# SerezD/vqvae-vqgan-pytorch-lightning

Measured on AMD Instinct MI355X. Metric: images/sec/node (256x256 bs=32/GPU) VQ-VAE train step, higher is better.
Workload: dtype bf16; 1 GPU; standard_vqvae cb=1024, 256x256 bs=32/GPU (encoder+VQ+decoder fwd/bwd + AdamW); yaml=example_confs/standard_vqvae.yaml, global_batch=32, parallelism=dp1, launch=hipGraph replay (fwd+bwd) + eager all-reduce + AdamW, deterministic=False

## Files before the change

include/vqk.h:

```cpp
#ifndef VQK_H_
#define VQK_H_

#include <stddef.h>
#include <stdint.h>

#ifdef __cplusplus
extern "C" {
#endif

#define VQK_F32 0
#define VQK_BF16 1

enum vqk_status {
    VQK_OK = 0,
    VQK_ERR_SHAPE = -1,
    VQK_ERR_DTYPE = -2,
    VQK_ERR_ALIGN = -3,
    VQK_ERR_LAUNCH = -4,
    VQK_ERR_ARG = -5,
    VQK_ERR_WORKSPACE = -6
};

const char* vqk_status_str(int status);
int vqk_version(void);
// ... 162 lines not shown
int vqk_ctx_set_tile_queue(vqk_ctx* ctx, void* ws, int64_t ws_bytes);
int vqk_ctx_set_deterministic(vqk_ctx* ctx, int on, void* ws, int64_t ws_bytes);
int vqk_set_tuning(const char* name, int value);
int vqk_reset_tuning(void);
int vqk_tuning_count(void);
const char* vqk_tuning_name(int i);
int vqk_conv_set_block_caps(int stream_blocks, int wgrad_blocks);
int vqk_probe_stream_add(const float* src, float* dst, int64_t bytes, int blocks, int passes, int sleep, void* stream);
int vqk_calib_fill(void* w, int64_t bytes, void* stream);
int vqk_calib_mfma(const void* w, int64_t w_bytes, float* sink, int iters, int blocks, void* stream);
int64_t vqk_calib_mfma_flops(int iters, int blocks);
int vqk_calib_copy(const void* src, void* dst, int64_t bytes, void* stream);
int vqk_conv_pack_dgrad(const float* w, void* wt, int dtype, int cout, int cin, int ksize, void* stream);
int vqk_conv2d_wgrad(int dtype, const void* x, const void* dy, float* dw, int n, int h_in, int w_in, int cin,
                     int cout, int ksize, int ups, const void* zeros, void* stream);
int64_t vqk_conv2d_wgrad_edge_ws_bytes(void);
int vqk_conv2d_wgrad_edge(int dtype, const void* x, const void* dy, float* dw, void* ws, int64_t ws_bytes, int n, int h,
                          int w, int cin, int cout, const void* zeros, void* stream);
int vqk_conv2d_wgrad_edge_true(int dtype, const void* x, const void* dy, float* dw, void* ws, int64_t ws_bytes, int n, int h,
                               int w, int cin, int cout, int thin_true, const void* zeros, void* stream);
int vqk_conv2d_thin_out(int dtype, const void* x, const void* w, const float* bias, void* y, int n, int h, int wd, int cin,
                        int cout, int act, const void* zeros, void* stream);
int vqk_colsum(int dtype, const void* x, int64_t rows, int c, float* out, void* stream);
int vqk_colsum_lead(int dtype, const void* x, int64_t rows, int c, int c_out, float scale, float* out, void* stream);
int vqk_cast(const float* src, void* dst, int dtype, int64_t n, void* stream);

int vqk_gn_stats(int dtype, const void* x, int n, int64_t hw, int c, int groups, float eps,
                 double* acc, float* stats, void* stream);
int vqk_gn_apply(int dtype, const void* x, const float* stats, const float* w, const float* b, void* y,
                 int n, int64_t hw, int c, int groups, int silu, void* stream);
int vqk_gn_forward(int dtype, const void* x, const float* w, const float* b, void* y, float* stats, double* ws, int n,
                   int64_t hw, int c, int groups, float eps, int silu, void* stream);
int vqk_gn_forward_presummed(int dtype, const void* x, const float* w, const float* b, void* y, float* stats, double* ws,
                             int n, int64_t hw, int c, int groups, float eps, int silu, void* stream);
int vqk_gn_forward_presummed_parts(int dtype, const void* x, const float* w, const float* b, void* y, float* stats,
// ... 130 lines not shown
```

vqvae-vqgan-pytorch-lightning_amd/_native.py:

```python
from __future__ import annotations

import ctypes
import fcntl
import os
import subprocess
from ctypes import c_char_p, c_double, c_float, c_int, c_int32, c_int64, c_void_p, POINTER

_HERE = os.path.dirname(os.path.abspath(__file__))
_CSRC = os.path.join(_HERE, 'csrc')
_SO = os.environ.get('VQK_LIB') or os.path.join(_HERE, 'libvqk.so')
_lib = None

P = c_void_p
I, L, F = c_int, c_int64, c_float

_PROTOS = {
    'vqk_row_sqnorm_f32': [P, L, I, P, P],
    'vqk_vq_assign_f32': [P, P, P, P, L, I, I, I, P, P],
    'vqk_vq_assign_filtered_f32': [P, P, P, P, L, I, I, I, P, P, L, P],
    'vqk_probe_stream_add': [P, P, L, I, I, I, P],
    'vqk_calib_fill': [P, L, P],
    'vqk_calib_mfma': [P, L, P, I, I, P],
    'vqk_calib_copy': [P, P, L, P],
    'vqk_vq_prepare_f32': [P, I, I, P, L, P],
# ... 51 lines not shown
    'vqk_conv_pack_weights': [P, P, I, I, I, I, I, I, P],
    'vqk_conv_pack_multi': [P, I, I, P],
    'vqk_conv_set_variant': [I],
    'vqk_conv_set_block_caps': [I, I],
    'vqk_set_deterministic': [I, P, L],
    'vqk_set_scratch': [P, L],
    'vqk_set_tile_queue': [P, L],
    'vqk_ctx_create': [P],
    'vqk_ctx_destroy': [P],
    'vqk_ctx_make_current': [P],
    'vqk_ctx_set_scratch': [P, P, L],
    'vqk_ctx_set_tile_queue': [P, P, L],
    'vqk_ctx_set_deterministic': [P, I, P, L],
    'vqk_conv_pack_dgrad': [P, P, I, I, I, I, P],
    'vqk_conv2d_wgrad': [I, P, P, P, I, I, I, I, I, I, I, P, P],
    'vqk_conv2d_wgrad_pooled_dy': [I, P, P, P, I, I, I, I, I, F, P, P],
    'vqk_conv2d_wgrad_ups_phase': [I, P, P, P, I, I, I, I, I, F, P, P],
    'vqk_split_pair_f32': [P, P, L, I, P],
    'vqk_conv2d_fprop_x3_gnstats': [P, P, P, P, P, I, I, I, I, I, I, P, I, P, P],
    'vqk_conv2d_wgrad_x3': [P, P, P, I, I, I, I, I, I, F, P, P],
    'vqk_conv2d_wgrad_x3_f32': [P, P, P, I, I, I, I, I, I, F, P],
    'vqk_conv2d_wgrad_pooled_dy_phase': [I, P, P, P, I, I, I, I, I, F, P, P],
    'vqk_conv2d_wgrad_edge': [I, P, P, P, P, L, I, I, I, I, I, P, P],
    'vqk_conv2d_wgrad_edge_true': [I, P, P, P, P, L, I, I, I, I, I, I, P, P],
    'vqk_conv2d_thin_out': [I, P, P, P, P, I, I, I, I, I, I, P, P],
    'vqk_colsum': [I, P, L, I, P, P],
    'vqk_colsum_lead': [I, P, L, I, I, F, P, P],
    'vqk_cast': [P, P, I, L, P],
    'vqk_gn_stats': [I, P, I, L, I, I, F, P, P, P],
    'vqk_gn_apply': [I, P, P, P, P, P, I, L, I, I, I, P],
    'vqk_gn_forward': [I, P, P, P, P, P, P, I, L, I, I, F, I, P],
    'vqk_gn_forward_presummed': [I, P, P, P, P, P, P, I, L, I, I, F, I, P],
    'vqk_gn_forward_presummed_parts': [I, P, P, P, P, P, P, I, P, I, L, I, I, F, I, P],
    'vqk_gn_backward': [I, P, P, P, P, P, P, P, P, P, I, L, I, I, I, I, P, P],
    'vqk_gn_backward_pooled_add': [I, P, P, P, P, P, P, P, P, P, I, I, I, I, I, I, P, F, P],
    'vqk_gn_backward_ws': [I, P, P, P, P, P, P, P, P, P, L, I, I, I, I, I, I, I, P, P, F, P],
    'vqk_gn_cluster_timeouts': [P],
    'vqk_gn_backward_colsum': [I, P, P, P, P, P, P, P, P, P, L, I, I, I, I, I, I, I, P, P, P],
    'vqk_pool2x2': [I, P, P, I, I, I, I, F, P],
# ... 124 lines not shown
```

vqvae-vqgan-pytorch-lightning_amd/csrc/api.cpp:

```cpp
#include <stdint.h>
#include <new>
#include "common.h"

extern "C" {

const char* vqk_status_str(int status) {
    switch (status) {
        case VQK_OK: return "ok";
        case VQK_ERR_SHAPE: return "unsupported or inconsistent shape";
        case VQK_ERR_DTYPE: return "unsupported dtype";
        case VQK_ERR_ALIGN: return "pointer is not 16-byte aligned";
        case VQK_ERR_LAUNCH: return "kernel launch failed";
        case VQK_ERR_ARG: return "bad argument";
        case VQK_ERR_WORKSPACE: return "workspace too small";
        default: return "unknown status";
    }
}

int vqk_version(void) { return 1; }
const char* vqk_arch(void) { return "gfx950"; }

}

struct vqk_ctx {
// ... 96 lines not shown
    {"GN_NO_SMALL", 0, 0},
    {"WGMX_COEF_E4", 0, 0},
    {"GN_CLUSTER_MAX_HW", 0, 0},
    {"COMM_CUS", 0, 0},
    {"MX_QUARTER", 0, 0},
    {"MX_S2", 0, 0},
    {"MX_S2_DGRAD_MIN", 0, 0},
    {"VQ_LDS", 0, 0},
    {"UPS_MERGE", 0, 0},
    {"TILE_QUEUE", 0, 0},
    {"X3_WL", 0, 0},
    {"X3_WGRAD_COEF_E4", 0, 0},
    {"X3_WGRAD_FOLD", 0, 0},
    {"X3_WGRAD_PHASE", 0, 0},
    {"X3_WGRAD_PHASE_CAP_PCT", 0, 0},
    {"X3_WGRAD_PHASE_COEF_E4", 0, 0}
};
static constexpr int kTune = (int)(sizeof(g_tune) / sizeof(g_tune[0]));
TuneSlot* tune_slot(const char* name) {
    for (int i = 0; i < kTune; ++i)
        if (strcmp(g_tune[i].name, name) == 0) return &g_tune[i];
    abort();
}
}

extern "C" int vqk_set_tuning(const char* name, int value) {
    if (!name) return VQK_ERR_ARG;
    for (int i = 0; i < vqkd::kTune; ++i)
        if (strcmp(vqkd::g_tune[i].name, name) == 0) {
            __atomic_store_n(&vqkd::g_tune[i].value, value, __ATOMIC_RELAXED);
            __atomic_store_n(&vqkd::g_tune[i].is_set, 1, __ATOMIC_RELEASE);
// ... 14 lines not shown
```

vqvae-vqgan-pytorch-lightning_amd/csrc/conv_edge.hip:

```cpp
#include "conv_geom.h"

namespace {

__device__ __forceinline__ void glds16(const void* src, char* lds_wave_base) {
    __builtin_amdgcn_global_load_lds((const VQK_GLB void*)src, (VQK_LDS void*)lds_wave_base, 16, 0, 0);
}

typedef __attribute__((ext_vector_type(8))) short s16x8;

template <int PITCH, bool SWZ>
__device__ __forceinline__ bf16x8_t tr_frag(const char* tile, int k0, int cbase, int lane) {
    const int i = lane & 15, grp = (lane >> 4) & 1, kgrp = lane >> 5;
    const int col = cbase + 16 * grp + 4 * (i & 3);
    const int row = k0 + 8 * kgrp + (i >> 2);
    const char* p0;
    if (SWZ) p0 = tile + row * PITCH + (((col >> 3) ^ ((row & 3) << 2)) << 4) + ((col & 7) << 1);
    else p0 = tile + row * PITCH + col * 2;
    const char* p1 = p0 + 4 * PITCH;
    const s16x4 lo = __builtin_amdgcn_ds_read_tr16_b64_v4i16((VQK_LDS s16x4*)p0);
    const s16x4 hi = __builtin_amdgcn_ds_read_tr16_b64_v4i16((VQK_LDS s16x4*)p1);
    const s16x8 v = {lo[0], lo[1], lo[2], lo[3], hi[0], hi[1], hi[2], hi[3]};
    return __builtin_bit_cast(bf16x8_t, v);
}

constexpr int EDGE_CW = 128;
constexpr int EDGE_PIX = 128;
constexpr int EDGE_WIDE_B = EDGE_PIX * EDGE_CW * 2;
constexpr int EDGE_IM_PITCH = 144;
constexpr int EDGE_IM_B = EDGE_PIX * EDGE_IM_PITCH;
constexpr int EDGE_STAGE = EDGE_WIDE_B + EDGE_IM_B;
constexpr int EDGE_LDS = 3 * EDGE_STAGE + 4096;
constexpr int EDGE_OUT = EDGE_CW * 72;

template <int MODE>
__global__ __launch_bounds__(256, 1) void conv3x3_wgrad_thin_kernel(const bf16_raw* __restrict__ wide,
                                                                    const bf16_raw* __restrict__ thin,
                                                                    float* __restrict__ ws, const char* __restrict__ zeros,
                                                                    int n, int h, int w) {
    extern __shared__ __attribute__((aligned(16))) char smem[];
    const int tid = threadIdx.x, lane = tid & 63;
    const int wave = __builtin_amdgcn_readfirstlane(tid >> 6);
    const int total = (int)(((int64_t)n * h * w) / EDGE_PIX);
    const int G = (int)gridDim.x, b = (int)blockIdx.x;
    const int cnt = (total - b + G - 1) / G;
    const int hw = h * w;
    constexpr int SGN = MODE == 0 ? 1 : -1;

    int s_ry[5], s_rx[5], s_ty[5], s_tx[5];
#pragma unroll
// ... 22 lines not shown
#pragma unroll
        for (int t = 0; t < 5; ++t) {
            const int q = wave + 4 * t;
            if (q < 18) {
                const int yy = y0 + s_ry[t] + s_ty[t], xx = x0 + s_rx[t] + s_tx[t];
                const void* src = zeros;
                if ((unsigned)yy < (unsigned)h && (unsigned)xx < (unsigned)w)
                    src = timg + ((int64_t)yy * w + xx) * 8;
                glds16(src, st + EDGE_WIDE_B + q * 1024);
            } else {
                glds16(zeros, smem + 3 * EDGE_STAGE + wave * 1024);
            }
        }
    };

    f32x16 acc[3];
#pragma unroll
    for (int j = 0; j < 3; ++j)
#pragma unroll
        for (int r = 0; r < 16; ++r) acc[j][r] = 0.0f;

    if (cnt > 0) issue(b, 0);
    if (cnt > 1) issue(b + G, 1);
    for (int i = 0; i < cnt; ++i) {
        if (i + 1 < cnt) asm volatile("s_waitcnt vmcnt(13)" ::: "memory");
        else asm volatile("s_waitcnt vmcnt(0)" ::: "memory");
        __syncthreads();
        if (i + 2 < cnt) issue(b + (i + 2) * G, (i + 2) % 3);
        const char* st = smem + (i % 3) * EDGE_STAGE;
#pragma unroll
        for (int k0 = 0; k0 < EDGE_PIX; k0 += 16) {
            const bf16x8_t a = tr_frag<EDGE_CW * 2, true>(st, k0, 32 * wave, lane);
#pragma unroll
            for (int j = 0; j < 3; ++j) {
                const bf16x8_t bj = tr_frag<EDGE_IM_PITCH, false>(st + EDGE_WIDE_B, k0, 32 * j, lane);
                acc[j] = __builtin_amdgcn_mfma_f32_32x32x16_bf16(a, bj, acc[j], 0, 0, 0);
            }
        }
    }
    float* part = ws + (int64_t)b * EDGE_OUT;
#pragma unroll
    for (int j = 0; j < 3; ++j) {
        const int col = 32 * j + (lane & 31);
        if (col >= 72) continue;
        const int tap = col >> 3, t = col & 7;
#pragma unroll
        for (int r = 0; r < 16; ++r) {
            const int wc = 32 * wave + (r & 3) + 8 * (r >> 2) + 4 * (lane >> 5);
            const int idx = MODE == 0 ? (wc * 9 + tap) * 8 + t : (t * 9 + tap) * EDGE_CW + wc;
            part[idx] = acc[j][r];
        }
    }
}

__global__ __launch_bounds__(256) void wgrad_thin_reduce_kernel(const float* __restrict__ ws, float* __restrict__ dw, int blocks,
                                                                int thin_true, int thin_in) {
    __shared__ float part[16][17];
    const int o = threadIdx.x & 15, kg = threadIdx.x >> 4;
    const int i = (int)blockIdx.x * 16 + o;
    float v[16];
#pragma unroll
    for (int j = 0; j < 16; ++j) {
        const int k = kg * 16 + j;
        v[j] = k < blocks ? ws[(int64_t)k * EDGE_OUT + i] : 0.0f;
    }
    float s = 0.0f;
#pragma unroll
    for (int j = 0; j < 16; ++j) s += v[j];
    part[kg][o] = s;
    __syncthreads();
    if (threadIdx.x < 16) {
        float t = 0.0f;
#pragma unroll
        for (int g2 = 0; g2 < 16; ++g2) t += part[g2][threadIdx.x];
        const int i2 = (int)blockIdx.x * 16 + (int)threadIdx.x;
        if (thin_true >= 8) dw[i2] += t;
        else if (thin_in) { const int ci = i2 & 7; if (ci < thin_true) dw[(i2 >> 3) * thin_true + ci] += t; }
        else if (i2 < thin_true * 9 * EDGE_CW) dw[i2] += t;
    }
}


constexpr int TO_TH = 8, TO_TW = 32, TO_HW2 = TO_TW + 2, TO_HPIX = (TO_TH + 2) * TO_HW2;
constexpr int TO_PITCH = 144, TO_PIECES = 48, TO_STAGE = TO_PIECES * 1024, TO_LDS = 2 * TO_STAGE;
typedef __attribute__((ext_vector_type(4))) unsigned int eu32x4;
typedef __attribute__((ext_vector_type(2))) unsigned int eu32x2;

__global__ __launch_bounds__(256, 1) void conv3x3_thin_out_kernel(const bf16_raw* __restrict__ x, const bf16_raw* __restrict__ wgt,
                                                                  const float* __restrict__ bias, bf16_raw* __restrict__ y,
                                                                  const char* __restrict__ zeros, int n, int h, int w, int act) {
    extern __shared__ __attribute__((aligned(16))) char smem[];
// ... 94 lines not shown
                    if (act == 1) v[e] = tanhf(v[e]);
                }
                const int yy = cur.y0 + 2 * wave + (gq >> 1), xx = cur.x0 + 16 * (gq & 1) + px;
                const eu32x2 o = {vqkd::pack_bf16x2(v[0], v[1]), vqkd::pack_bf16x2(v[2], v[3])};
                *reinterpret_cast<eu32x2*>(y + (((int64_t)cur.img * h + yy) * w + xx) * 8 + 4 * kq) = o;
            }
        }
        cur = nxt;
    }
}

}

extern "C" {

int64_t vqk_conv2d_wgrad_edge_ws_bytes(void) { return (int64_t)256 * EDGE_OUT * 4; }

int vqk_conv2d_wgrad_edge(int dtype, const void* x, const void* dy, float* dw, void* ws, int64_t ws_bytes, int n, int h,
                          int w, int cin, int cout, const void* zeros, void* stream) {
    return vqk_conv2d_wgrad_edge_true(dtype, x, dy, dw, ws, ws_bytes, n, h, w, cin, cout, 8, zeros, stream);
}

int vqk_conv2d_wgrad_edge_true(int dtype, const void* x, const void* dy, float* dw, void* ws, int64_t ws_bytes, int n, int h,
                               int w, int cin, int cout, int thin_true, const void* zeros, void* stream) {
    VQK_REQUIRE(x && dy && dw && ws && zeros, VQK_ERR_ARG);
    VQK_REQUIRE(thin_true >= 1 && thin_true <= 8, VQK_ERR_ARG);
    VQK_REQUIRE(vqk_aligned16(x) && vqk_aligned16(dy) && vqk_aligned16(ws) && vqk_aligned16(zeros), VQK_ERR_ALIGN);
    VQK_REQUIRE(dtype == VQK_BF16, VQK_ERR_DTYPE);
    VQK_REQUIRE(n > 0 && h > 0 && w > 0, VQK_ERR_SHAPE);
    const bool first = cin == 8 && cout == EDGE_CW, last = cout == 8 && cin == EDGE_CW;
    const int64_t m = (int64_t)n * h * w;
    VQK_REQUIRE((first || last) && ((int64_t)h * w) % EDGE_PIX == 0 && (w % EDGE_PIX == 0 || EDGE_PIX % w == 0) && m < 0x7fffffffLL,
                VQK_ERR_SHAPE);
    const int total = (int)(m / EDGE_PIX);
    int blocks = total < 256 ? total : 256;
    VQK_REQUIRE(ws_bytes >= (int64_t)blocks * EDGE_OUT * 4, VQK_ERR_ARG);
    hipStream_t st = vqk_stream(stream);
    if (first) {
        static const hipError_t attr = hipFuncSetAttribute((const void*)conv3x3_wgrad_thin_kernel<0>,
                                                           hipFuncAttributeMaxDynamicSharedMemorySize, EDGE_LDS);
        if (attr != hipSuccess) return VQK_ERR_LAUNCH;
        hipLaunchKernelGGL(conv3x3_wgrad_thin_kernel<0>, dim3((unsigned)blocks), dim3(256), EDGE_LDS, st, (const bf16_raw*)dy,
                           (const bf16_raw*)x, (float*)ws, (const char*)zeros, n, h, w);
    } else {
        static const hipError_t attr = hipFuncSetAttribute((const void*)conv3x3_wgrad_thin_kernel<1>,
                                                           hipFuncAttributeMaxDynamicSharedMemorySize, EDGE_LDS);
        if (attr != hipSuccess) return VQK_ERR_LAUNCH;
        hipLaunchKernelGGL(conv3x3_wgrad_thin_kernel<1>, dim3((unsigned)blocks), dim3(256), EDGE_LDS, st, (const bf16_raw*)x,
                           (const bf16_raw*)dy, (float*)ws, (const char*)zeros, n, h, w);
    }
    VQK_CHECK_LAUNCH();
    static_assert(EDGE_OUT % 16 == 0, "reduce blocks own 16 outputs");
    hipLaunchKernelGGL(wgrad_thin_reduce_kernel, dim3(EDGE_OUT / 16), dim3(256), 0, st, (const float*)ws, dw, blocks, thin_true, first ? 1 : 0);
    VQK_CHECK_LAUNCH();
    return VQK_OK;
}

int vqk_conv2d_thin_out(int dtype, const void* x, const void* w, const float* bias, void* y, int n, int h, int wd, int cin,
                        int cout, int act, const void* zeros, void* stream) {
    VQK_REQUIRE(x && w && y && zeros, VQK_ERR_ARG);
    VQK_REQUIRE(vqk_aligned16(x) && vqk_aligned16(w) && vqk_aligned16(y) && vqk_aligned16(zeros), VQK_ERR_ALIGN);
    VQK_REQUIRE(dtype == VQK_BF16, VQK_ERR_DTYPE);
    VQK_REQUIRE(act == 0 || act == 1, VQK_ERR_ARG);
    VQK_REQUIRE(n > 0 && cin == 128 && cout == 8 && h > 0 && wd > 0 && (h % TO_TH) == 0 && (wd % TO_TW) == 0 &&
                (int64_t)n * h * wd * 128 * 2 < 0x7fffffff0LL, VQK_ERR_SHAPE);
    const int total = n * (h / TO_TH) * (wd / TO_TW);
    const int blocks = total < 256 ? total : 256;
    static const hipError_t attr = hipFuncSetAttribute((const void*)conv3x3_thin_out_kernel,
// ... 10 lines not shown
```

vqvae-vqgan-pytorch-lightning_amd/ops.py:

```python
from __future__ import annotations

import os
import threading
import weakref

import numpy as _np
import torch

from . import _native

F32, BF16 = 0, 1
_CL = torch.channels_last


def dcode(dtype: torch.dtype) -> int:
    if dtype == torch.float32:
        return F32
    if dtype == torch.bfloat16:
        return BF16
    raise RuntimeError(f'vqk: unsupported dtype {dtype}')


def epc(dtype: torch.dtype) -> int:
    return 4 if dtype == torch.float32 else 8
# ... 722 lines not shown
    return _tagged((tensor,), lambda: tensor.backward(*args, **kwargs))


def autograd_grad(outputs, inputs, *args, **kwargs):
    roots = outputs if isinstance(outputs, (tuple, list)) else (outputs,)
    return _tagged(roots, lambda: torch.autograd.grad(outputs, inputs, *args, **kwargs))


def direct_grad(param):
    if _grad_modes()[0] and getattr(param, '_vqk_direct_grad', False) and param.grad is not None:
        return param.grad
    return None


_EDGE_WGRAD = _native.switch('VQK_EDGE_WGRAD', '1') != '0'
_EDGE_WS: dict = {}


def _edge_ws(device) -> torch.Tensor:
    _stream()
    key = _wkey(device)
    ws = _EDGE_WS.get(key)
    if ws is None:
        ws = _EDGE_WS[key] = torch.empty(_native.lib().vqk_conv2d_wgrad_edge_ws_bytes() // 4, dtype=torch.float32, device=device)
    return ws


def edge_wgrad_served(x, dy, ksize: int, ups: bool) -> bool:
    n, cin, h, w = x.shape
    return (_EDGE_WGRAD and x.dtype == torch.bfloat16 and ksize == 3 and not ups and (cin, dy.shape[1]) in ((8, 128), (128, 8))
            and (h * w) % 128 == 0 and (w % 128 == 0 or 128 % w == 0))


def raw_split_pair(t) -> torch.Tensor:
    n, c, h, w = t.shape
    out = empty_nhwc(n, 2 * c, h, w, torch.bfloat16, t.device)
    st = _timed('split_pair_kernel (HBM)', 0.0,
                lambda: _native.lib().vqk_split_pair_f32(t.data_ptr(), out.data_ptr(), n * h * w, c, _stream()), t.numel() * 8.0)
    _native.check(st, 'split_pair')
    return out


def raw_conv_wgrad(x, dy, ksize: int, ups: bool, out=None, thin_true: int = 8, x3: bool = False) -> torch.Tensor:
    n, cin, h, w = x.shape
    cout = dy.shape[1]
    dw = out if out is not None else \
        torch.zeros((cout, ksize, ksize, cin), dtype=torch.float32, device=x.device).permute(0, 3, 1, 2)
    flops = 2.0 * n * dy.shape[2] * dy.shape[3] * cout * cin * ksize * ksize
    if edge_wgrad_served(x, dy, ksize, ups):
        ws = _edge_ws(x.device)
        nbytes = (x.numel() + dy.numel()) * 2
        st = _timed('conv3x3_wgrad_thin_kernel<bf16>' + (f' {cin}->{cout}@{h}x{w}' if _EVENT_SHAPES else ''), 0.0,
                    lambda: _native.lib().vqk_conv2d_wgrad_edge_true(dcode(x.dtype), x.data_ptr(), dy.data_ptr(), dw.data_ptr(),
                                                                     ws.data_ptr(), ws.numel() * 4, n, h, w, cin, cout, int(thin_true),
                                                                     zero_page(x.device).data_ptr(), _stream()), nbytes)
        _native.check(st, 'conv2d_wgrad_edge')
        return dw
    if thin_true != 8:
        raise RuntimeError('vqk: an unpadded weight-gradient target needs the edge-conv kernel')
    if (x3 and not X3_WGRAD_FOLD and x.dtype == torch.float32 and dy.dtype == torch.float32 and ksize == 3 and cin % 64 == 0
            and cout % 64 == 0 and dy.shape[3] % 8 == 0 and dy.shape[2] % 8 == 0 and not DETERMINISTIC):
        phase = bool(ups) and X3_WGRAD_PHASE and h % 8 == 0 and w % 8 == 0
        st = _timed('conv3x3_wgrad_x3_kernel<f32 as 3 x bf16>' + (f' {cin}->{cout}@{dy.shape[2]}x{dy.shape[3]} k3{" phase" if phase else ""}' if _EVENT_SHAPES else ''), flops,
                    lambda: _native.lib().vqk_conv2d_wgrad_x3_f32(x.data_ptr(), dy.data_ptr(), dw.data_ptr(), n, h, w, cin, cout, int(ups),
                                                                  1.0, _stream()), exec_flops=3.0 * flops * (4.0 / 9.0 if phase else 1.0))
        if st != _native.ERR_SHAPE:
            _native.check(st, 'conv2d_wgrad_x3_f32')
            return dw
    if (x3 and x.dtype == torch.float32 and dy.dtype == torch.float32 and ksize == 3 and cin % 64 == 0 and cout % 64 == 0
            and dy.shape[3] % 16 == 0 and dy.shape[2] % 8 == 0 and not DETERMINISTIC and _WGMX_ON):
        xp, dyp = raw_split_pair(x), raw_split_pair(dy)
        st = _timed('conv3x3_wgrad_mx_kernel<f32 as 3 x bf16>' + (f' {cin}->{cout}@{dy.shape[2]}x{dy.shape[3]} k3' if _EVENT_SHAPES else ''), flops,
                    lambda: _native.lib().vqk_conv2d_wgrad_x3(xp.data_ptr(), dyp.data_ptr(), dw.data_ptr(), n, h, w, cin, cout, int(ups),
                                                              1.0, zero_page(x.device).data_ptr(), _stream()), exec_flops=3.0 * flops)
# ... 648 lines not shown
            n_img, _, h_out, w_out = dyc.shape
            layout = weight_layout(dt, n_img, h_out, w_out, cout_pad, cin, k, False, x3=ctx.x3)
            if ups and ctx.phase and UPS_PHASE == 1:
                dx = raw_conv_ups_phase(dyc, packed_weight(weight, cin, cout_pad, dt, k, True, phase_layout(dt, ctx.x3)), None, cin, True)
            if dx is not None:
                pass
            elif ups and can_pool_epilogue(dt, cin, layout):
                wt = packed_weight(weight, cin, cout_pad, dt, k, True, layout)
                dx = raw_conv_fprop_pooled(dyc, wt, None, None, k, False, cin, 1.0)
            else:
                wt = packed_weight(weight, cin, cout_pad, dt, k, True, layout)
                dx = raw_conv_fprop(dyc, wt, None, None, k, False, 0, dt, cin, layout)
                if ups:
                    dx = raw_pool(dx, 1.0)
        padded = cin != i or cout_pad != o
        if ctx.needs_input_grad[1]:
            tgt = None if padded else direct_grad(ctx.weight_ref)
            thin = 8
            if padded and edge_wgrad_served(x, dyc, k, ups) and (cin == i or cout_pad == o):
                tgt = direct_grad(ctx.weight_ref)
                thin = (i if cin != i else o) if tgt is not None else 8
            dw = raw_conv_wgrad(x, dyc, k, ups, out=tgt, thin_true=thin, x3=ctx.x3)
            if tgt is not None:
                dw = None
            elif padded:
                dw = dw[:o, :i]
        if has_bias and ctx.needs_input_grad[2] and id(ctx.bias_ref) in _DB_DONE:
            _DB_DONE.discard(id(ctx.bias_ref))
        elif has_bias and ctx.needs_input_grad[2]:
            n, c, h, w = dyc.shape
            tgt = direct_grad(ctx.bias_ref) if (cout_pad == c) else None
            db = raw_colsum(n * h * w, c, dyc, out=tgt, lead=o if tgt is not None else None)
            db = None if tgt is not None else db[:o]
        return dx, dw, db, dres, None, None, None, None


def conv2d(x, weight, bias=None, residual=None, ups: bool = False, act: int = 0, out_dtype=None, next_gn: int = 0):
    return Conv2dFn.apply(x, weight, bias, residual, ups, act, out_dtype, next_gn)


class GroupNormSiLUFn(torch.autograd.Function):

# ... 353 lines not shown
```

Before: 1165 images/sec.

## Add streaming 1x1 conv wgrad kernel and fuse bias-gradient sums into wgrad

Adds a new split-K MFMA kernel for 1x1 convolution weight gradients that streams pixels through LDS. It picks the pixel split heuristically and folds the partial sums, or writes atomically. Both this kernel and the thin edge 3x3 wgrad kernel now compute the bias gradient in the same pass by multiplying against a ones vector. This removes the separate colsum launch and its second read of dy. The cost is extra MFMA work and workspace, and the edge workspace size grows.

```diff
diff --git a/include/vqk.h b/include/vqk.h
--- a/include/vqk.h
+++ b/include/vqk.h
@@ -200,11 +200,16 @@
 int vqk_conv_pack_dgrad(const float* w, void* wt, int dtype, int cout, int cin, int ksize, void* stream);
 int vqk_conv2d_wgrad(int dtype, const void* x, const void* dy, float* dw, int n, int h_in, int w_in, int cin,
                      int cout, int ksize, int ups, const void* zeros, void* stream);
+int vqk_conv2d_wgrad_1x1_served(int cin, int cout);
+int vqk_conv2d_wgrad_1x1(const void* x, const void* dy, float* dw, float* db, int64_t pixels, int cin, int cout, int splits,
+                         const void* zeros, void* stream);
 int64_t vqk_conv2d_wgrad_edge_ws_bytes(void);
 int vqk_conv2d_wgrad_edge(int dtype, const void* x, const void* dy, float* dw, void* ws, int64_t ws_bytes, int n, int h,
                           int w, int cin, int cout, const void* zeros, void* stream);
 int vqk_conv2d_wgrad_edge_true(int dtype, const void* x, const void* dy, float* dw, void* ws, int64_t ws_bytes, int n, int h,
                                int w, int cin, int cout, int thin_true, const void* zeros, void* stream);
+int vqk_conv2d_wgrad_edge_db(int dtype, const void* x, const void* dy, float* dw, float* db, void* ws, int64_t ws_bytes, int n, int h,
+                             int w, int cin, int cout, int thin_true, const void* zeros, void* stream);
 int vqk_conv2d_thin_out(int dtype, const void* x, const void* w, const float* bias, void* y, int n, int h, int wd, int cin,
                         int cout, int act, const void* zeros, void* stream);
 int vqk_colsum(int dtype, const void* x, int64_t rows, int c, float* out, void* stream);
diff --git a/vqvae-vqgan-pytorch-lightning_amd/_native.py b/vqvae-vqgan-pytorch-lightning_amd/_native.py
--- a/vqvae-vqgan-pytorch-lightning_amd/_native.py
+++ b/vqvae-vqgan-pytorch-lightning_amd/_native.py
@@ -89,6 +89,8 @@
     'vqk_ctx_set_deterministic': [P, I, P, L],
     'vqk_conv_pack_dgrad': [P, P, I, I, I, I, P],
     'vqk_conv2d_wgrad': [I, P, P, P, I, I, I, I, I, I, I, P, P],
+    'vqk_conv2d_wgrad_1x1': [P, P, P, P, L, I, I, I, P, P],
+    'vqk_conv2d_wgrad_1x1_served': [I, I],
     'vqk_conv2d_wgrad_pooled_dy': [I, P, P, P, I, I, I, I, I, F, P, P],
     'vqk_conv2d_wgrad_ups_phase': [I, P, P, P, I, I, I, I, I, F, P, P],
     'vqk_split_pair_f32': [P, P, L, I, P],
@@ -98,6 +100,7 @@
     'vqk_conv2d_wgrad_pooled_dy_phase': [I, P, P, P, I, I, I, I, I, F, P, P],
     'vqk_conv2d_wgrad_edge': [I, P, P, P, P, L, I, I, I, I, I, P, P],
     'vqk_conv2d_wgrad_edge_true': [I, P, P, P, P, L, I, I, I, I, I, I, P, P],
+    'vqk_conv2d_wgrad_edge_db': [I, P, P, P, P, P, L, I, I, I, I, I, I, P, P],
     'vqk_conv2d_thin_out': [I, P, P, P, P, I, I, I, I, I, I, P, P],
     'vqk_colsum': [I, P, L, I, P, P],
     'vqk_colsum_lead': [I, P, L, I, I, F, P, P],
diff --git a/vqvae-vqgan-pytorch-lightning_amd/csrc/api.cpp b/vqvae-vqgan-pytorch-lightning_amd/csrc/api.cpp
--- a/vqvae-vqgan-pytorch-lightning_amd/csrc/api.cpp
+++ b/vqvae-vqgan-pytorch-lightning_amd/csrc/api.cpp
@@ -134,7 +134,10 @@
     {"X3_WGRAD_FOLD", 0, 0},
     {"X3_WGRAD_PHASE", 0, 0},
     {"X3_WGRAD_PHASE_CAP_PCT", 0, 0},
-    {"X3_WGRAD_PHASE_COEF_E4", 0, 0}
+    {"X3_WGRAD_PHASE_COEF_E4", 0, 0},
+    {"PIXRED_BLOCKS", 0, 0},
+    {"PIXRED_COEF", 0, 0},
+    {"PIXRED_ATOMIC", 0, 0}
 };
 static constexpr int kTune = (int)(sizeof(g_tune) / sizeof(g_tune[0]));
 TuneSlot* tune_slot(const char* name) {
diff --git a/vqvae-vqgan-pytorch-lightning_amd/csrc/conv_edge.hip b/vqvae-vqgan-pytorch-lightning_amd/csrc/conv_edge.hip
--- a/vqvae-vqgan-pytorch-lightning_amd/csrc/conv_edge.hip
+++ b/vqvae-vqgan-pytorch-lightning_amd/csrc/conv_edge.hip
@@ -31,8 +31,10 @@
 constexpr int EDGE_STAGE = EDGE_WIDE_B + EDGE_IM_B;
 constexpr int EDGE_LDS = 3 * EDGE_STAGE + 4096;
 constexpr int EDGE_OUT = EDGE_CW * 72;
-
-template <int MODE>
+constexpr int EDGE_MAXB = 256;
+constexpr int EDGE_DBW = 128;
+
+template <int MODE, bool DB>
 __global__ __launch_bounds__(256, 1) void conv3x3_wgrad_thin_kernel(const bf16_raw* __restrict__ wide,
                                                                     const bf16_raw* __restrict__ thin,
                                                                     float* __restrict__ ws, const char* __restrict__ zeros,
@@ -85,11 +87,16 @@
         }
     };
 
-    f32x16 acc[3];
+    f32x16 acc[3], accb;
 #pragma unroll
     for (int j = 0; j < 3; ++j)
 #pragma unroll
         for (int r = 0; r < 16; ++r) acc[j][r] = 0.0f;
+#pragma unroll
+    for (int r = 0; r < 16; ++r) accb[r] = 0.0f;
+    bf16x8_t ones;
+#pragma unroll
+    for (int e = 0; e < 8; ++e) ones[e] = (__bf16)1.0f;
 
     if (cnt > 0) issue(b, 0);
     if (cnt > 1) issue(b + G, 1);
@@ -106,7 +113,9 @@
             for (int j = 0; j < 3; ++j) {
                 const bf16x8_t bj = tr_frag<EDGE_IM_PITCH, false>(st + EDGE_WIDE_B, k0, 32 * j, lane);
                 acc[j] = __builtin_amdgcn_mfma_f32_32x32x16_bf16(a, bj, acc[j], 0, 0, 0);
-            }
+                if (DB && MODE == 1 && j == 1 && wave == 0) accb = __builtin_amdgcn_mfma_f32_32x32x16_bf16(ones, bj, accb, 0, 0, 0);
+            }
+            if (DB && MODE == 0) accb = __builtin_amdgcn_mfma_f32_32x32x16_bf16(a, ones, accb, 0, 0, 0);
         }
     }
     float* part = ws + (int64_t)b * EDGE_OUT;
@@ -122,18 +131,32 @@
             part[idx] = acc[j][r];
         }
     }
+    if (DB) {
+        float* pdb = ws + (int64_t)EDGE_MAXB * EDGE_OUT + (int64_t)b * EDGE_DBW;
+        if (MODE == 0) {
+            if ((lane & 31) == 0) {
+#pragma unroll
+                for (int r = 0; r < 16; ++r) pdb[32 * wave + (r & 3) + 8 * (r >> 2) + 4 * (lane >> 5)] = accb[r];
+            }
+        } else if (wave == 0 && lane < 8) {
+            pdb[lane] = accb[0];
+        }
+    }
 }
 
 __global__ __launch_bounds__(256) void wgrad_thin_reduce_kernel(const float* __restrict__ ws, float* __restrict__ dw, int blocks,
-                                                                int thin_true, int thin_in) {
+                                                                int thin_true, int thin_in, float* __restrict__ db, int db_count) {
     __shared__ float part[16][17];
     const int o = threadIdx.x & 15, kg = threadIdx.x >> 4;
-    const int i = (int)blockIdx.x * 16 + o;
+    const bool isdb = (int)blockIdx.x >= EDGE_OUT / 16;
+    const int i = (isdb ? (int)blockIdx.x - EDGE_OUT / 16 : (int)blockIdx.x) * 16 + o;
+    const float* src = isdb ? ws + (int64_t)EDGE_MAXB * EDGE_OUT : ws;
+    const int pitch = isdb ? EDGE_DBW : EDGE_OUT;
     float v[16];
 #pragma unroll
     for (int j = 0; j < 16; ++j) {
         const int k = kg * 16 + j;
-        v[j] = k < blocks ? ws[(int64_t)k * EDGE_OUT + i] : 0.0f;
+        v[j] = k < blocks ? src[(int64_t)k * pitch + i] : 0.0f;
     }
     float s = 0.0f;
 #pragma unroll
@@ -144,8 +167,9 @@
         float t = 0.0f;
 #pragma unroll
         for (int g2 = 0; g2 < 16; ++g2) t += part[g2][threadIdx.x];
-        const int i2 = (int)blockIdx.x * 16 + (int)threadIdx.x;
-        if (thin_true >= 8) dw[i2] += t;
+        const int i2 = (isdb ? (int)blockIdx.x - EDGE_OUT / 16 : (int)blockIdx.x) * 16 + (int)threadIdx.x;
+        if (isdb) { if (i2 < db_count) db[i2] += t; }
+        else if (thin_true >= 8) dw[i2] += t;
         else if (thin_in) { const int ci = i2 & 7; if (ci < thin_true) dw[(i2 >> 3) * thin_true + ci] += t; }
         else if (i2 < thin_true * 9 * EDGE_CW) dw[i2] += t;
     }
@@ -270,7 +294,7 @@
 
 extern "C" {
 
-int64_t vqk_conv2d_wgrad_edge_ws_bytes(void) { return (int64_t)256 * EDGE_OUT * 4; }
+int64_t vqk_conv2d_wgrad_edge_ws_bytes(void) { return (int64_t)EDGE_MAXB * (EDGE_OUT + EDGE_DBW) * 4; }
 
 int vqk_conv2d_wgrad_edge(int dtype, const void* x, const void* dy, float* dw, void* ws, int64_t ws_bytes, int n, int h,
                           int w, int cin, int cout, const void* zeros, void* stream) {
@@ -279,6 +303,11 @@
 
 int vqk_conv2d_wgrad_edge_true(int dtype, const void* x, const void* dy, float* dw, void* ws, int64_t ws_bytes, int n, int h,
                                int w, int cin, int cout, int thin_true, const void* zeros, void* stream) {
+    return vqk_conv2d_wgrad_edge_db(dtype, x, dy, dw, nullptr, ws, ws_bytes, n, h, w, cin, cout, thin_true, zeros, stream);
+}
+
+int vqk_conv2d_wgrad_edge_db(int dtype, const void* x, const void* dy, float* dw, float* db, void* ws, int64_t ws_bytes, int n, int h,
+                             int w, int cin, int cout, int thin_true, const void* zeros, void* stream) {
     VQK_REQUIRE(x && dy && dw && ws && zeros, VQK_ERR_ARG);
     VQK_REQUIRE(thin_true >= 1 && thin_true <= 8, VQK_ERR_ARG);
     VQK_REQUIRE(vqk_aligned16(x) && vqk_aligned16(dy) && vqk_aligned16(ws) && vqk_aligned16(zeros), VQK_ERR_ALIGN);
@@ -289,25 +318,27 @@
     VQK_REQUIRE((first || last) && ((int64_t)h * w) % EDGE_PIX == 0 && (w % EDGE_PIX == 0 || EDGE_PIX % w == 0) && m < 0x7fffffffLL,
                 VQK_ERR_SHAPE);
     const int total = (int)(m / EDGE_PIX);
-    int blocks = total < 256 ? total : 256;
-    VQK_REQUIRE(ws_bytes >= (int64_t)blocks * EDGE_OUT * 4, VQK_ERR_ARG);
+    int blocks = total < EDGE_MAXB ? total : EDGE_MAXB;
+    VQK_REQUIRE(ws_bytes >= (db ? vqk_conv2d_wgrad_edge_ws_bytes() : (int64_t)blocks * EDGE_OUT * 4), VQK_ERR_ARG);
     hipStream_t st = vqk_stream(stream);
+#define VQK_EDGE_LAUNCH(MODE, DB, WIDE, THIN)                                                                                      \
+    do {                                                                                                                          \
+        static const hipError_t attr = hipFuncSetAttribute((const void*)conv3x3_wgrad_thin_kernel<MODE, DB>,                      \
+                                                           hipFuncAttributeMaxDynamicSharedMemorySize, EDGE_LDS);                 \
+        if (attr != hipSuccess) return VQK_ERR_LAUNCH;                                                                            \
+        hipLaunchKernelGGL((conv3x3_wgrad_thin_kernel<MODE, DB>), dim3((unsigned)blocks), dim3(256), EDGE_LDS, st,                \
+                           (const bf16_raw*)(WIDE), (const bf16_raw*)(THIN), (float*)ws, (const char*)zeros, n, h, w);            \
+    } while (0)
     if (first) {
-        static const hipError_t attr = hipFuncSetAttribute((const void*)conv3x3_wgrad_thin_kernel<0>,
-                                                           hipFuncAttributeMaxDynamicSharedMemorySize, EDGE_LDS);
-        if (attr != hipSuccess) return VQK_ERR_LAUNCH;
-        hipLaunchKernelGGL(conv3x3_wgrad_thin_kernel<0>, dim3((unsigned)blocks), dim3(256), EDGE_LDS, st, (const bf16_raw*)dy,
-                           (const bf16_raw*)x, (float*)ws, (const char*)zeros, n, h, w);
+        if (db) VQK_EDGE_LAUNCH(0, true, dy, x); else VQK_EDGE_LAUNCH(0, false, dy, x);
     } else {
-        static const hipError_t attr = hipFuncSetAttribute((const void*)conv3x3_wgrad_thin_kernel<1>,
-                                                           hipFuncAttributeMaxDynamicSharedMemorySize, EDGE_LDS);
-        if (attr != hipSuccess) return VQK_ERR_LAUNCH;
-        hipLaunchKernelGGL(conv3x3_wgrad_thin_kernel<1>, dim3((unsigned)blocks), dim3(256), EDGE_LDS, st, (const bf16_raw*)x,
-                           (const bf16_raw*)dy, (float*)ws, (const char*)zeros, n, h, w);
-    }
+        if (db) VQK_EDGE_LAUNCH(1, true, x, dy); else VQK_EDGE_LAUNCH(1, false, x, dy);
+    }
+#undef VQK_EDGE_LAUNCH
     VQK_CHECK_LAUNCH();
-    static_assert(EDGE_OUT % 16 == 0, "reduce blocks own 16 outputs");
-    hipLaunchKernelGGL(wgrad_thin_reduce_kernel, dim3(EDGE_OUT / 16), dim3(256), 0, st, (const float*)ws, dw, blocks, thin_true, first ? 1 : 0);
+    static_assert(EDGE_OUT % 16 == 0 && EDGE_DBW % 16 == 0, "reduce blocks own 16 outputs");
+    hipLaunchKernelGGL(wgrad_thin_reduce_kernel, dim3(EDGE_OUT / 16 + (db ? EDGE_DBW / 16 : 0)), dim3(256), 0, st, (const float*)ws, dw,
+                       blocks, thin_true, first ? 1 : 0, db, first ? EDGE_CW : thin_true);
     VQK_CHECK_LAUNCH();
     return VQK_OK;
 }
diff --git a/vqvae-vqgan-pytorch-lightning_amd/csrc/conv_wgrad_1x1.hip b/vqvae-vqgan-pytorch-lightning_amd/csrc/conv_wgrad_1x1.hip
--- /dev/null
+++ b/vqvae-vqgan-pytorch-lightning_amd/csrc/conv_wgrad_1x1.hip
@@ -0,0 +1,265 @@
+#include "common.h"
+#include <math.h>
+
+namespace {
+
+__device__ __forceinline__ void glds16(const void* src, char* lds_wave_base) {
+    __builtin_amdgcn_global_load_lds((const VQK_GLB void*)src, (VQK_LDS void*)lds_wave_base, 16, 0, 0);
+}
+
+template <int ROWB>
+__device__ __forceinline__ bf16x8_t tr_frag(const char* tile, int k0, int cbase, int lane) {
+    constexpr int SH = ROWB == 256 ? 2 : 1;
+    const int i = lane & 15, grp = (lane >> 4) & 1, kgrp = lane >> 5;
+    const int col = cbase + 16 * grp + 4 * (i & 3);
+    const int row = k0 + 8 * kgrp + (i >> 2);
+    const int lc = col >> 3;
+    const char* p0 = tile + row * ROWB + ((lc ^ ((row & 3) << SH)) << 4) + ((col & 7) << 1);
+    const char* p1 = p0 + 4 * ROWB;
+    const s16x4 lo = __builtin_amdgcn_ds_read_tr16_b64_v4i16((VQK_LDS s16x4*)p0);
+    const s16x4 hi = __builtin_amdgcn_ds_read_tr16_b64_v4i16((VQK_LDS s16x4*)p1);
+    typedef __attribute__((ext_vector_type(8))) short s16x8;
+    const s16x8 v = {lo[0], lo[1], lo[2], lo[3], hi[0], hi[1], hi[2], hi[3]};
+    return __builtin_bit_cast(bf16x8_t, v);
+}
+
+template <int TCO, int TCI, int WM, int WN, bool DB>
+__global__ __launch_bounds__(512) void conv1x1_wgrad_stream_kernel(const bf16_raw* __restrict__ x, const bf16_raw* __restrict__ dy,
+                                                                   float* __restrict__ dw, float* __restrict__ db,
+                                                                   float* __restrict__ part, const char* __restrict__ zeros, int m,
+                                                                   int cin, int cout, int pix_per_split, int64_t slice_stride) {
+    constexpr int KP = (TCO + TCI) > 384 ? 32 : 64;
+    constexpr int KW = 8 / (WM * WN), MI = TCO / WM / 32, NJ = TCI / WN / 32;
+    constexpr int SWA = TCO < 128 ? 64 : 128, SWB = TCI < 128 ? 64 : 128;
+    constexpr int ROWBA = SWA * 2, ROWBB = SWB * 2;
+    constexpr int A_BYTES = KP * TCO * 2, B_BYTES = KP * TCI * 2, STAGE = A_BYTES + B_BYTES;
+    constexpr int PA = A_BYTES / 1024, PB = B_BYTES / 1024, NL = (PA + PB) / 8;
+    static_assert((PA + PB) % 8 == 0 && KP / 16 >= KW && MI >= 1 && NJ >= 1, "tile shape");
+    extern __shared__ __attribute__((aligned(16))) char smem[];
+    const int tid = threadIdx.x, lane = tid & 63;
+    const int wave = __builtin_amdgcn_readfirstlane(tid >> 6);
+    const int kq = wave / (WM * WN), wm = (wave % (WM * WN)) / WN, wn = wave % WN;
+    const int co0 = cout > TCO ? (int)blockIdx.x * TCO : 0;
+    const int ci0 = cin > TCI ? (int)blockIdx.x * TCI : 0;
+    const int p_begin = (int)blockIdx.y * pix_per_split;
+    const int p_end = min(m, p_begin + pix_per_split);
+    const int nsteps = (p_end - p_begin + KP - 1) / KP;
+
+    unsigned s_off[NL];
+    int s_row[NL];
+#pragma unroll
+    for (int t = 0; t < NL; ++t) {
+        const int q = wave + 8 * t;
+        const bool isa = q < PA;
+        const int ql = isa ? q : q - PA;
+        const int rowb = isa ? ROWBA : ROWBB, cpr = rowb >> 4, rpp = 1024 / rowb, pps = KP / rpp;
+        const int sub = ql / pps, pr = ql - sub * pps;
+        const int row = pr * rpp + lane / cpr, pc = lane % cpr;
+        const int lc = pc ^ ((row & 3) << (cpr == 16 ? 2 : 1));
+        const int ch = (isa ? co0 : ci0) + sub * (rowb >> 1) + lc * 8;
+        s_row[t] = row;
+        s_off[t] = (unsigned)((row * (isa ? cout : cin) + ch) * 2);
+    }
+    auto issue = [&](int step, char* st) {
+        const int p0 = p_begin + step * KP;
+        const bool full = p0 + KP <= p_end;
+        const char* ba = reinterpret_cast<const char*>(dy) + (int64_t)p0 * cout * 2;
+        const char* bb = reinterpret_cast<const char*>(x) + (int64_t)p0 * cin * 2;
+#pragma unroll
+        for (int t = 0; t < NL; ++t) {
+            const int q = wave + 8 * t;
+            const char* src = (q < PA ? ba : bb) + s_off[t];
+            if (!full && p0 + s_row[t] >= p_end) src = zeros;
+            glds16(src, st + q * 1024);
+        }
+    };
+
+    f32x16 acc[MI][NJ];
+    f32x16 accb[MI];
+#pragma unroll
+    for (int i = 0; i < MI; ++i) {
+#pragma unroll
+        for (int j = 0; j < NJ; ++j)
+#pragma unroll
+            for (int r = 0; r < 16; ++r) acc[i][j][r] = 0.0f;
+#pragma unroll
+        for (int r = 0; r < 16; ++r) accb[i][r] = 0.0f;
+    }
+    bf16x8_t ones;
+#pragma unroll
+    for (int e = 0; e < 8; ++e) ones[e] = (__bf16)1.0f;
+    const bool do_db = DB && wn == 0 && ci0 == 0;
+
+    if (nsteps > 0) issue(0, smem);
+    if (nsteps > 1) issue(1, smem + STAGE);
+    int cur = 0;
+    for (int it = 0; it < nsteps; ++it) {
+        if (it + 1 < nsteps) asm volatile("s_waitcnt vmcnt(%0)" ::"n"(NL) : "memory");
+        else asm volatile("s_waitcnt vmcnt(0)" ::: "memory");
+        asm volatile("s_waitcnt lgkmcnt(0)\n\ts_barrier" ::: "memory");
+        const int nxt2 = cur == 0 ? 2 : cur - 1;
+        if (it + 2 < nsteps) issue(it + 2, smem + nxt2 * STAGE);
+        const char* lds_a = smem + cur * STAGE;
+        const char* lds_b = lds_a + A_BYTES;
+#pragma unroll
+        for (int ks = 0; ks < KP / 16 / KW; ++ks) {
+            const int k0 = (ks * KW + kq) * 16;
+            bf16x8_t a[MI], b[NJ];
+#pragma unroll
+            for (int i = 0; i < MI; ++i) {
+                const int cl = (wm * MI + i) * 32;
+                a[i] = tr_frag<ROWBA>(lds_a + (cl / SWA) * (KP * ROWBA), k0, cl % SWA, lane);
+            }
+#pragma unroll
+            for (int j = 0; j < NJ; ++j) {
+                const int cl = (wn * NJ + j) * 32;
+                b[j] = tr_frag<ROWBB>(lds_b + (cl / SWB) * (KP * ROWBB), k0, cl % SWB, lane);
+            }
+#pragma unroll
+            for (int i = 0; i < MI; ++i) {
+#pragma unroll
+                for (int j = 0; j < NJ; ++j) acc[i][j] = __builtin_amdgcn_mfma_f32_32x32x16_bf16(a[i], b[j], acc[i][j], 0, 0, 0);
+                if (DB && do_db) accb[i] = __builtin_amdgcn_mfma_f32_32x32x16_bf16(a[i], ones, accb[i], 0, 0, 0);
+            }
+        }
+        cur = cur == 2 ? 0 : cur + 1;
+    }
+
+    const int64_t dw_elems = (int64_t)cout * cin;
+    const int co_l = co0 + wm * MI * 32 + 4 * (lane >> 5);
+    const int64_t lane_o = (int64_t)co_l * cin + ci0 + wn * NJ * 32 + (lane & 31);
+    if (part) {
+        float* slice = part + ((int64_t)blockIdx.y * KW + kq) * slice_stride;
+#pragma unroll
+        for (int i = 0; i < MI; ++i)
+#pragma unroll
+            for (int r = 0; r < 16; ++r) {
+                const int row = i * 32 + (r & 3) + 8 * (r >> 2);
+#pragma unroll
+                for (int j = 0; j < NJ; ++j) slice[lane_o + (int64_t)row * cin + j * 32] = acc[i][j][r];
+                if (DB && do_db && (lane & 31) == 0) slice[dw_elems + co_l + row] = accb[i][r];
+            }
+    } else {
+#pragma unroll
+        for (int i = 0; i < MI; ++i)
+#pragma unroll
+            for (int r = 0; r < 16; ++r) {
+                const int row = i * 32 + (r & 3) + 8 * (r >> 2);
+#pragma unroll
+                for (int j = 0; j < NJ; ++j) atomicAdd(dw + lane_o + (int64_t)row * cin + j * 32, acc[i][j][r]);
+                if (DB && do_db && (lane & 31) == 0) atomicAdd(db + co_l + row, accb[i][r]);
+            }
+    }
+}
+
+__global__ __launch_bounds__(1024) void conv1x1_wgrad_fold_kernel(const float* __restrict__ part, int64_t slice_stride, int slices,
+                                                                  int64_t dw_elems, int64_t total, float* __restrict__ dw,
+                                                                  float* __restrict__ db) {
+    __shared__ f32x4 red[16][64];
+    const int lane = threadIdx.x & 63, w = threadIdx.x >> 6;
+    const int64_t e = ((int64_t)blockIdx.x * 64 + lane) * 4;
+    f32x4 s = {0.f, 0.f, 0.f, 0.f};
+    if (e < total) {
+        const float* p = part + e;
+        int k = w;
+        for (; k + 48 < slices; k += 64) {
+            const f32x4 v0 = *reinterpret_cast<const f32x4*>(p + (int64_t)k * slice_stride);
+            const f32x4 v1 = *reinterpret_cast<const f32x4*>(p + (int64_t)(k + 16) * slice_stride);
+            const f32x4 v2 = *reinterpret_cast<const f32x4*>(p + (int64_t)(k + 32) * slice_stride);
+            const f32x4 v3 = *reinterpret_cast<const f32x4*>(p + (int64_t)(k + 48) * slice_stride);
+            s += v0; s += v1; s += v2; s += v3;
+        }
+        for (; k < slices; k += 16) s += *reinterpret_cast<const f32x4*>(p + (int64_t)k * slice_stride);
+    }
+    red[w][lane] = s;
+    __syncthreads();
+    if (w == 0 && e < total) {
+        f32x4 t = red[0][lane];
+#pragma unroll
+        for (int k = 1; k < 16; ++k) t += red[k][lane];
+        float* d = e < dw_elems ? dw + e : db + (e - dw_elems);
+        f32x4 o = *reinterpret_cast<f32x4*>(d);
+        o += t;
+        *reinterpret_cast<f32x4*>(d) = o;
+    }
+}
+
+template <int TCO, int TCI, int WM, int WN>
+int launch_stream(const void* x, const void* dy, float* dw, float* db, float* part, const void* zeros, int m, int cin, int cout,
+                  int groups, int splits, int pps, int64_t slice_stride, hipStream_t st) {
+    constexpr int KP = (TCO + TCI) > 384 ? 32 : 64;
+    constexpr int lds = 3 * (TCO + TCI) * KP * 2;
+    const dim3 grid((unsigned)groups, (unsigned)splits);
+    if (db) {
+        static const hipError_t attr = hipFuncSetAttribute((const void*)conv1x1_wgrad_stream_kernel<TCO, TCI, WM, WN, true>,
+                                                           hipFuncAttributeMaxDynamicSharedMemorySize, lds);
+        if (attr != hipSuccess) return VQK_ERR_LAUNCH;
+        hipLaunchKernelGGL((conv1x1_wgrad_stream_kernel<TCO, TCI, WM, WN, true>), grid, dim3(512), lds, st, (const bf16_raw*)x,
+                           (const bf16_raw*)dy, dw, db, part, (const char*)zeros, m, cin, cout, pps, slice_stride);
+    } else {
+        static const hipError_t attr = hipFuncSetAttribute((const void*)conv1x1_wgrad_stream_kernel<TCO, TCI, WM, WN, false>,
+                                                           hipFuncAttributeMaxDynamicSharedMemorySize, lds);
+        if (attr != hipSuccess) return VQK_ERR_LAUNCH;
+        hipLaunchKernelGGL((conv1x1_wgrad_stream_kernel<TCO, TCI, WM, WN, false>), grid, dim3(512), lds, st, (const bf16_raw*)x,
+                           (const bf16_raw*)dy, dw, db, part, (const char*)zeros, m, cin, cout, pps, slice_stride);
+    }
+    return VQK_OK;
+}
+
+}
+
+extern "C" int vqk_conv2d_wgrad_1x1_served(int cin, int cout) {
+    const int tco = cout > 256 ? 256 : cout, tci = cin > 256 ? 256 : cin;
+    if (cout > 512 || cin > 512 || (cout > 256 && cin > 256)) return 0;
+    return (tco == 64 && tci == 64) || (tco == 128 && tci == 128) || (tco == 256 && tci == 128) || (tco == 128 && tci == 256) ||
+           (tco == 256 && tci == 256);
+}
+
+extern "C" int vqk_conv2d_wgrad_1x1(const void* x, const void* dy, float* dw, float* db, int64_t pixels, int cin, int cout,
+                                    int splits, const void* zeros, void* stream) {
+    VQK_REQUIRE(x && dy && dw && zeros, VQK_ERR_ARG);
+    VQK_REQUIRE(vqk_aligned16(x) && vqk_aligned16(dy) && vqk_aligned16(zeros) && vqk_aligned16(dw) && (!db || vqk_aligned16(db)), VQK_ERR_ALIGN);
+    VQK_REQUIRE(pixels > 0 && pixels < 0x7fff0000 && splits >= 0, VQK_ERR_ARG);
+    VQK_REQUIRE(vqk_conv2d_wgrad_1x1_served(cin, cout) && vqkd::det_state().on == 0, VQK_ERR_SHAPE);
+    const int m = (int)pixels;
+    const int tco = cout > 256 ? 256 : cout, tci = cin > 256 ? 256 : cin;
+    const int groups = (cout / tco) * (cin / tci);
+    const int kp = (tco + tci) > 384 ? 32 : 64;
+    const int kw = (tco == 64 && tci == 64) ? 4 : (tco == 128 && tci == 128) ? 2 : 1;
+    const int64_t dw_elems = (int64_t)cout * cin, slice_stride = dw_elems + cout;
+    const vqkd::DetState& sc = vqkd::scratch_state();
+    if (splits == 0) {
+        const double bytes = (double)m * (cin + cout) * 2.0, tile_bytes = (double)tco * tci * 4.0;
+        const int cap = VQK_TUNE("PIXRED_BLOCKS", 256);
+        int blocks = (int)(sqrt((double)VQK_TUNE("PIXRED_COEF", 140) * bytes / tile_bytes) + 0.5);
+        if (blocks > cap) blocks = cap;
+        splits = blocks / groups;
+        if (splits > m / (2 * kp)) splits = m / (2 * kp);
+    }
+    if (splits < 1) splits = 1;
+    float* part = nullptr;
+    if (splits > 1 && sc.ws && !VQK_TUNE("PIXRED_ATOMIC", 0)) {
+        const int64_t fit = sc.bytes / (slice_stride * 4 * kw);
+        if (splits > fit) splits = (int)fit;
+        if (splits > 1) part = sc.ws;
+    }
+    int pps = (m + splits - 1) / splits;
+    pps = (pps + kp - 1) / kp * kp;
+    splits = (m + pps - 1) / pps;
+    if (splits < 2) part = nullptr;
+    hipStream_t st = vqk_stream(stream);
+    int rc;
+    if (tco == 64) rc = launch_stream<64, 64, 2, 1>(x, dy, dw, db, part, zeros, m, cin, cout, groups, splits, pps, slice_stride, st);
+    else if (tco == 128 && tci == 128) rc = launch_stream<128, 128, 2, 2>(x, dy, dw, db, part, zeros, m, cin, cout, groups, splits, pps, slice_stride, st);
+    else if (tco == 256 && tci == 128) rc = launch_stream<256, 128, 4, 2>(x, dy, dw, db, part, zeros, m, cin, cout, groups, splits, pps, slice_stride, st);
+    else if (tco == 128 && tci == 256) rc = launch_stream<128, 256, 2, 4>(x, dy, dw, db, part, zeros, m, cin, cout, groups, splits, pps, slice_stride, st);
+    else rc = launch_stream<256, 256, 4, 2>(x, dy, dw, db, part, zeros, m, cin, cout, groups, splits, pps, slice_stride, st);
+    if (rc) return rc;
+    if (part) {
+        const int64_t total = dw_elems + (db ? cout : 0);
+        hipLaunchKernelGGL(conv1x1_wgrad_fold_kernel, dim3((unsigned)((total / 4 + 63) / 64)), dim3(1024), 0, st, (const float*)part,
+                           slice_stride, splits * kw, dw_elems, total, dw, db);
+    }
+    VQK_CHECK_LAUNCH();
+    return VQK_OK;
+}
diff --git a/vqvae-vqgan-pytorch-lightning_amd/ops.py b/vqvae-vqgan-pytorch-lightning_amd/ops.py
--- a/vqvae-vqgan-pytorch-lightning_amd/ops.py
+++ b/vqvae-vqgan-pytorch-lightning_amd/ops.py
@@ -760,6 +760,7 @@
 
 
 _EDGE_WGRAD = _native.switch('VQK_EDGE_WGRAD', '1') != '0'
+_EDGE_DB = _native.switch('VQK_EDGE_DB', '1') != '0'
 _EDGE_WS: dict = {}
 
 
@@ -787,7 +788,17 @@
     return out
 
 
-def raw_conv_wgrad(x, dy, ksize: int, ups: bool, out=None, thin_true: int = 8, x3: bool = False) -> torch.Tensor:
+PIXRED_1X1 = _native.switch('VQK_PIXRED_1X1', '1') != '0'
+
+
+def pixred_1x1_served(x, dy, ksize: int, ups: bool) -> bool:
+    cin, cout = x.shape[1], dy.shape[1]
+    return (PIXRED_1X1 and ksize == 1 and not ups and not DETERMINISTIC and x.dtype == torch.bfloat16 and dy.dtype == torch.bfloat16
+            and cin % 64 == 0 and cout % 64 == 0 and tuple(x.shape[2:]) == tuple(dy.shape[2:])
+            and _native.lib().vqk_conv2d_wgrad_1x1_served(cin, cout) == 1)
+
+
+def raw_conv_wgrad(x, dy, ksize: int, ups: bool, out=None, thin_true: int = 8, x3: bool = False, db=None, splits: int = 0) -> torch.Tensor:
     n, cin, h, w = x.shape
     cout = dy.shape[1]
     dw = out if out is not None else \
@@ -797,13 +808,22 @@
         ws = _edge_ws(x.device)
         nbytes = (x.numel() + dy.numel()) * 2
         st = _timed('conv3x3_wgrad_thin_kernel<bf16>' + (f' {cin}->{cout}@{h}x{w}' if _EVENT_SHAPES else ''), 0.0,
-                    lambda: _native.lib().vqk_conv2d_wgrad_edge_true(dcode(x.dtype), x.data_ptr(), dy.data_ptr(), dw.data_ptr(),
-                                                                     ws.data_ptr(), ws.numel() * 4, n, h, w, cin, cout, int(thin_true),
-                                                                     zero_page(x.device).data_ptr(), _stream()), nbytes)
+                    lambda: _native.lib().vqk_conv2d_wgrad_edge_db(dcode(x.dtype), x.data_ptr(), dy.data_ptr(), dw.data_ptr(), _p(db),
+                                                                   ws.data_ptr(), ws.numel() * 4, n, h, w, cin, cout, int(thin_true),
+                                                                   zero_page(x.device).data_ptr(), _stream()), nbytes)
         _native.check(st, 'conv2d_wgrad_edge')
         return dw
     if thin_true != 8:
         raise RuntimeError('vqk: an unpadded weight-gradient target needs the edge-conv kernel')
+    if pixred_1x1_served(x, dy, ksize, ups):
+        st = _timed('conv1x1_wgrad_stream_kernel<bf16>' + (f' {cin}->{cout}@{h}x{w} k1' if _EVENT_SHAPES else ''), flops,
+                    lambda: _native.lib().vqk_conv2d_wgrad_1x1(x.data_ptr(), dy.data_ptr(), dw.data_ptr(), _p(db), n * h * w, cin, cout,
+                                                               int(splits), zero_page(x.device).data_ptr(), _stream()),
+                    (x.numel() + dy.numel()) * 2)
+        _native.check(st, 'conv2d_wgrad_1x1')
+        return dw
+    if db is not None:
+        raise RuntimeError('vqk: a fused bias sum needs the streaming 1x1 weight-gradient kernel')
     if (x3 and not X3_WGRAD_FOLD and x.dtype == torch.float32 and dy.dtype == torch.float32 and ksize == 3 and cin % 64 == 0
             and cout % 64 == 0 and dy.shape[3] % 8 == 0 and dy.shape[2] % 8 == 0 and not DETERMINISTIC):
         phase = bool(ups) and X3_WGRAD_PHASE and h % 8 == 0 and w % 8 == 0
@@ -1482,18 +1502,35 @@
                 if ups:
                     dx = raw_pool(dx, 1.0)
         padded = cin != i or cout_pad != o
+        db_fused, db_direct = None, False
         if ctx.needs_input_grad[1]:
             tgt = None if padded else direct_grad(ctx.weight_ref)
             thin = 8
             if padded and edge_wgrad_served(x, dyc, k, ups) and (cin == i or cout_pad == o):
                 tgt = direct_grad(ctx.weight_ref)
                 thin = (i if cin != i else o) if tgt is not None else 8
-            dw = raw_conv_wgrad(x, dyc, k, ups, out=tgt, thin_true=thin, x3=ctx.x3)
+            if (has_bias and ctx.needs_input_grad[2] and id(ctx.bias_ref) not in _DB_DONE and not padded
+                    and pixred_1x1_served(x, dyc, k, ups)):
+                db_fused = direct_grad(ctx.bias_ref)
+                db_direct = db_fused is not None
+                if not db_direct:
+                    db_fused = torch.zeros(o, dtype=torch.float32, device=dyc.device)
+            elif (has_bias and ctx.needs_input_grad[2] and id(ctx.bias_ref) not in _DB_DONE and _EDGE_DB
+                    and edge_wgrad_served(x, dyc, k, ups)):
+                count = cout_pad if cin == 8 else thin
+                dgb = direct_grad(ctx.bias_ref)
+                if dgb is not None and count == o:
+                    db_fused, db_direct = dgb, True
+                elif dgb is None:
+                    db_fused = torch.zeros(count, dtype=torch.float32, device=dyc.device)
+            dw = raw_conv_wgrad(x, dyc, k, ups, out=tgt, thin_true=thin, x3=ctx.x3, db=db_fused)
             if tgt is not None:
                 dw = None
             elif padded:
                 dw = dw[:o, :i]
-        if has_bias and ctx.needs_input_grad[2] and id(ctx.bias_ref) in _DB_DONE:
+        if db_fused is not None:
+            db = None if db_direct else db_fused[:o]
+        elif has_bias and ctx.needs_input_grad[2] and id(ctx.bias_ref) in _DB_DONE:
             _DB_DONE.discard(id(ctx.bias_ref))
         elif has_bias and ctx.needs_input_grad[2]:
             n, c, h, w = dyc.shape
```

Result: no change. 1164 images/sec (-0.1%).
